# RaphaelHaddad/Real-Time-Brain-Inspired-Video-Memory

Measured on NVIDIA B200. Metric: queries_per_sec_top10_384d, higher is better.
Workload: dtype tf32

## Files before the change

real-time-brain-inspired-video-memory_b200/csrc/common.cuh:

```cuda
#pragma once
#include <cuda_runtime.h>
#include <cuda_bf16.h>
#include <stdint.h>
#include <stdio.h>
#include <math.h>
#include <utility>
#include "../../include/vidmem.h"

namespace vm {

void set_error(const char *fmt, ...);
#define VM_CUDA_CHECK(expr)                                                                      \
    do {                                                                                         \
        cudaError_t _e = (expr);                                                                 \
        if (_e != cudaSuccess) {                                                                 \
            vm::set_error("%s failed: %s (%s:%d)", #expr, cudaGetErrorString(_e), __FILE__, __LINE__); \
            return VM_ERR_CUDA;                                                                  \
        }                                                                                        \
    } while (0)
#define VM_REQUIRE(cond, code, ...)          \
    do {                                     \
        if (!(cond)) {                       \
            vm::set_error(__VA_ARGS__);      \
            return (code);                   \
        }                                    \
    } while (0)

__device__ __forceinline__ void pdl_wait() { asm volatile("griddepcontrol.wait;" ::: "memory"); }
__device__ __forceinline__ void pdl_launch_dependents() { asm volatile("griddepcontrol.launch_dependents;" ::: "memory"); }

template <typename... KArgs, typename... Args>
static inline cudaError_t launch_pdl(void (*kernel)(KArgs...), dim3 grid, dim3 block, size_t smem, cudaStream_t st, bool pdl,
                                     Args &&...args)
{
    cudaLaunchConfig_t cfg = {};
    cfg.gridDim = grid; cfg.blockDim = block; cfg.dynamicSmemBytes = smem; cfg.stream = st;
    cudaLaunchAttribute at[1];
    at[0].id = cudaLaunchAttributeProgrammaticStreamSerialization;
    at[0].val.programmaticStreamSerializationAllowed = 1;
    cfg.attrs = at;
    cfg.numAttrs = pdl ? 1 : 0;
    return cudaLaunchKernelEx(&cfg, kernel, std::forward<Args>(args)...);
}

template <auto Kernel>
static inline cudaError_t max_smem_once(int bytes)
{
    static bool set[64] = {};
    int dev = 0;
    cudaError_t e = cudaGetDevice(&dev);
    if (e != cudaSuccess || set[dev & 63]) return e;
    e = cudaFuncSetAttribute(Kernel, cudaFuncAttributeMaxDynamicSharedMemorySize, bytes);
    if (e == cudaSuccess) set[dev & 63] = true;
    return e;
}

__host__ __device__ __forceinline__ uint32_t f32_ordered(float f)
{
#ifdef __CUDA_ARCH__
    uint32_t b = __float_as_uint(f);
#else
    uint32_t b;
    memcpy(&b, &f, 4);
#endif
    return (b & 0x80000000u) ? ~b : (b | 0x80000000u);
}
__host__ __device__ __forceinline__ float f32_from_ordered(uint32_t o)
{
    uint32_t b = (o & 0x80000000u) ? (o & 0x7FFFFFFFu) : ~o;
#ifdef __CUDA_ARCH__
    return __uint_as_float(b);
#else
    float f;
    memcpy(&f, &b, 4);
    return f;
#endif
}
__host__ __device__ __forceinline__ uint64_t make_key(float score, uint32_t row)
{
    return ((uint64_t)f32_ordered(score) << 32) | (uint64_t)(0xFFFFFFFFu - row);
}
__host__ __device__ __forceinline__ uint32_t key_row(uint64_t k) { return 0xFFFFFFFFu - (uint32_t)(k & 0xFFFFFFFFu); }
__host__ __device__ __forceinline__ float key_score(uint64_t k) { return f32_from_ordered((uint32_t)(k >> 32)); }

static constexpr int SEED_TAB_WORDS = 256 * 64;
#ifdef __CUDACC__
__device__ __forceinline__ float seed_select(const uint32_t *seed_tab, int G, int nq_pad, int q, int k, int lane)
{
    uint32_t vals[8];
#pragma unroll
    for (int t = 0; t < 8; ++t) {
        const int i = lane + 32 * t;
        vals[t] = i < G ? __ldcg(seed_tab + (size_t)i * nq_pad + q) : 0u;
    }
    uint32_t prefix = 0;
    int need = k;
    for (int bit = 31; bit >= 16; --bit) {
        const uint32_t hi = bit == 31 ? 0u : (0xFFFFFFFFu << (bit + 1));
        int cnt = 0;
#pragma unroll
        for (int t = 0; t < 8; ++t) cnt += ((vals[t] & hi) == prefix && ((vals[t] >> bit) & 1u)) ? 1 : 0;
        const int tot = __reduce_add_sync(0xffffffffu, cnt);
        if (tot >= need) prefix |= 1u << bit;
        else need -= tot;
    }
    float sd = f32_from_ordered(prefix);
    if (!(sd > -INFINITY) || G < k) sd = -INFINITY;
    return sd;
}

__device__ __forceinline__ float band_floor(float L, float band)
{
    if (!(L > -INFINITY)) return -INFINITY;
    const float t = __fsub_rd(L, band);
    return nextafterf(t, -INFINITY);
}

#endif

struct RefSum {
    double s, c;
    __device__ __forceinline__ void init() { s = 0.0; c = 0.0; }
    template <bool NEUMAIER>
    __device__ __forceinline__ void add(double x)
    {
        double t = __dadd_rn(s, x);
        if (NEUMAIER) {
            const bool big = fabs(s) >= fabs(x);
            const double hi = big ? s : x, lo = big ? x : s;
            c = __dadd_rn(c, __dadd_rn(__dadd_rn(hi, -t), lo));
        }
        s = t;
    }
    template <bool NEUMAIER>
    __device__ __forceinline__ void add_block(const double (&x)[8])
    {
        double t[8];
        t[0] = __dadd_rn(s, x[0]);
#pragma unroll
        for (int u = 1; u < 8; ++u) t[u] = __dadd_rn(t[u - 1], x[u]);
        if (NEUMAIER) {
#pragma unroll
            for (int u = 0; u < 8; ++u) {
                const double prev = u ? t[u - 1] : s;
                const bool big = fabs(prev) >= fabs(x[u]);
                const double hi = big ? prev : x[u], lo = big ? x[u] : prev;
                c = __dadd_rn(c, __dadd_rn(__dadd_rn(hi, -t[u]), lo));
            }
        }
        s = t[7];
    }
    template <bool NEUMAIER>
    __device__ __forceinline__ double result() const
    {
        double r = s;
        if (NEUMAIER && c != 0.0 && isfinite(c)) r = __dadd_rn(r, c);
        return r;
    }
};

template <bool NEUMAIER, typename F>
__device__ __forceinline__ void ref_sum_range(RefSum &acc, int lo, int hi, F prod)
{
    int i = lo;
    for (; i + 8 <= hi; i += 8) {
        double x[8];
#pragma unroll
        for (int u = 0; u < 8; ++u) x[u] = prod(i + u);
        acc.add_block<NEUMAIER>(x);
    }
    for (; i < hi; ++i) acc.add<NEUMAIER>(prod(i));
}

__device__ __forceinline__ float load_as_float(const float *p, int64_t i) { return p[i]; }
__device__ __forceinline__ float load_as_float(const __nv_bfloat16 *p, int64_t i) { return __bfloat162float(p[i]); }
__device__ __forceinline__ double load_elem(const float *p, int64_t i) { return (double)p[i]; }
__device__ __forceinline__ double load_elem(const __nv_bfloat16 *p, int64_t i) { return (double)__bfloat162float(p[i]); }
__device__ __forceinline__ double load_elem(const double *p, int64_t i) { return p[i]; }
__device__ __forceinline__ double load_as_double(const void *p, int dtype, int64_t i)
{
    if (dtype == VM_F32) return (double)((const float *)p)[i];
    if (dtype == VM_BF16) return (double)__bfloat162float(((const __nv_bfloat16 *)p)[i]);
    return ((const double *)p)[i];
}

static inline int64_t imin64(int64_t a, int64_t b) { return a < b ? a : b; }
static inline int ld_for_dim(int dim) { return (dim + 7) & ~7; }
static inline size_t dtype_size(int dt) { return dt == VM_F32 ? 4 : dt == VM_BF16 ? 2 : 8; }

struct ScanArgs {
    const void *rows;
    const float *inv_norms;
    int dtype;
    int64_t n;
    int dim, ld;
    const float *queries;
    int nq;
    int kp;
    uint64_t *cand;
    int ctas;
    cudaStream_t stream;
    int dump = 0;
    uint64_t *slab = nullptr;
    int *scnt = nullptr;
    uint64_t *ubuf = nullptr;
    int *ucnt = nullptr;
    int ucap = 0;
    float band = 0.0f;
    int ksel = 0;
    int split = 0;
    bool pdl = false;
};
static constexpr int SCAN_UNION_CAP = 16384;
static constexpr int SCAN_SLAB = 128;
static constexpr int SELECT_KEY_CAP = 4096;
static constexpr int SCAN_DUMP_TILE = 128;
static constexpr int SCAN_DUMP_MAX_KEYS = 9472;
int launch_scan_simt(const ScanArgs &a);
int scan_simt_max_queries();
struct ScanCollect {
    const float *thr;
    uint64_t *buf;
    int *cnt;
    int cap;
    const int *pending;
};
struct ScanInfo { int stages = 0, variant = 0; };
int launch_scan_tc(const ScanArgs &a, const void *queries_store_dtype, uint32_t *seed_tab, int *seed_ctr,
                   const ScanCollect *sc = nullptr, ScanInfo *info = nullptr);
bool scan_tc_supported(int dtype, int dim, int nq, int kp, int split = 0);


struct FinalizeArgs {
    int k;
    double min_score;
    int score_mode;
    int64_t row_offset;
    int64_t *out_idx;
    double *out_score;
    int32_t *out_count;
};
struct RescoreArgs {
    const uint64_t *merged;
    int kp;
    const void *rows;
    const float *inv_norms;
    int dtype, ld, dim;
    int64_t n_rows;
    const void *queries;
    int q_dtype, nq;
    double eps;
    int sum_mode;
    FinalizeArgs fin;
    int32_t *flags, *uncertified_count;
    const int *extreme;
    float *collect_thr;
    unsigned long long *cum = nullptr;
};
struct SelectArgs {
    const uint64_t *cand = nullptr;
    int lists = 0, list_len = 0;
    int complete = 0;
    const uint64_t *slab = nullptr;
    const int *scnt = nullptr;
    int ctas = 0;
    const uint64_t *ubuf = nullptr;
    const int *ucnt = nullptr;
    int ucap = 0;
    const uint32_t *seed_tab = nullptr;
    int nq_pad = 0, ksel = 0;
    float band = 0.0f;
};
struct ExactArgs {
    const void *rows;
    const float *inv_norms;
    int dtype, ld, dim;
    int64_t n;
    const void *queries;
    int q_dtype, nq, k, sum_mode;
    int32_t *flags;
    double *xlist_score;
    uint32_t *xlist_row;
    int32_t *xlist_cnt;
    uint8_t *taken;
    int ctas;
    FinalizeArgs fin;
    unsigned long long *cum = nullptr;
    int *done_ctr = nullptr;
};

}
```

real-time-brain-inspired-video-memory_b200/csrc/select.cu:

```cuda
#include "common.cuh"

#include <type_traits>

namespace vm {

static constexpr int MERGE_THREADS = 512;
static constexpr int MERGE_SURV = 1024;

__device__ uint64_t radix_select_kth(const uint64_t *skeys, int total, int kp, int *hist, int *s_bin, int *s_need)
{
    const int tid = threadIdx.x, lane = tid & 31;
    uint64_t prefix = 0;
    int need = kp;
    for (int pass = 0; pass < 8; ++pass) {
        const int shift = 56 - 8 * pass;
        const uint64_t hmask = pass == 0 ? 0ull : (~0ull << (shift + 8));
        if (tid < 256) hist[tid] = 0;
        __syncthreads();
        for (int e = tid; e < total; e += MERGE_THREADS) {
            const uint64_t k = skeys[e];
            const bool act = k != 0 && (k & hmask) == prefix;
            const int bin = act ? (int)((k >> shift) & 0xFF) : -1;
            const unsigned peers = __match_any_sync(__activemask(), bin);
            if (act && (__ffs(peers) - 1) == lane) atomicAdd(&hist[bin], __popc(peers));
// ... 111 lines not shown
            if (nonzero >= kp && k == T) merged[(int64_t)q * kp + kp - 1] = k;
            else merged[(int64_t)q * kp + atomicAdd(&s_m, 1)] = k;
        }
    }
    __syncthreads();
    const int filled = s_m;
    const int last = nonzero >= kp ? kp - 1 : kp;
    for (int e = filled + tid; e < last; e += MERGE_THREADS) merged[(int64_t)q * kp + e] = 0;
}


__device__ __forceinline__ double convert_score(double c, int score_mode)
{
    return score_mode == VM_SCORE_NEO4J ? __ddiv_rn(__dadd_rn(1.0, c), 2.0) : c;
}

template <bool NEUMAIER, typename T>
__device__ double exact_cosine(const void *q, int q_dtype, int64_t qoff, const T *row, int dim)
{
    RefSum dot, qq, rr;
    dot.init(); qq.init(); rr.init();
    for (int i = 0; i < dim; ++i) {
        double x = load_as_double(q, q_dtype, qoff + i);
        double y = load_elem(row, i);
        dot.add<NEUMAIER>(__dmul_rn(x, y));
        qq.add<NEUMAIER>(__dmul_rn(x, x));
        rr.add<NEUMAIER>(__dmul_rn(y, y));
    }
    double n1 = __dsqrt_rn(qq.result<NEUMAIER>());
    double n2 = __dsqrt_rn(rr.result<NEUMAIER>());
    if (n1 == 0.0 || n2 == 0.0) return 0.0;
    return __ddiv_rn(dot.result<NEUMAIER>(), __dmul_rn(n1, n2));
}

template <bool NEUMAIER, typename T>
__device__ double exact_cosine_sq(const double *sq, double n1, const T *row, int dim)
{
    RefSum dot, rr;
    dot.init(); rr.init();
    ref_sum_range<NEUMAIER>(dot, 0, dim, [&](int i) { return __dmul_rn(sq[i], load_elem(row, i)); });
    ref_sum_range<NEUMAIER>(rr, 0, dim, [&](int i) { const double y = load_elem(row, i); return __dmul_rn(y, y); });
    double n2 = __dsqrt_rn(rr.result<NEUMAIER>());
    if (n1 == 0.0 || n2 == 0.0) return 0.0;
    return __ddiv_rn(dot.result<NEUMAIER>(), __dmul_rn(n1, n2));
}

__device__ __forceinline__ bool better(double sa, uint32_t ra, double sb, uint32_t rb)
{
    return sa > sb || (sa == sb && ra < rb);
}

static constexpr int RS_THREADS = 256;
static constexpr int RS_SMEM_ROW_BYTES = 96 * 1024;

__device__ __forceinline__ void load_vec16(const float *p, float *o)
{
    const float4 t = *reinterpret_cast<const float4 *>(p);
    o[0] = t.x; o[1] = t.y; o[2] = t.z; o[3] = t.w;
}
__device__ __forceinline__ void load_vec16(const __nv_bfloat16 *p, float *o)
{
    const uint4 u = *reinterpret_cast<const uint4 *>(p);
    o[0] = __uint_as_float(u.x << 16); o[1] = __uint_as_float(u.x & 0xffff0000u);
    o[2] = __uint_as_float(u.y << 16); o[3] = __uint_as_float(u.y & 0xffff0000u);
    o[4] = __uint_as_float(u.z << 16); o[5] = __uint_as_float(u.z & 0xffff0000u);
    o[6] = __uint_as_float(u.w << 16); o[7] = __uint_as_float(u.w & 0xffff0000u);
}

__device__ __forceinline__ void load_vec16(const double *p, double *o)
{
    const double2 t = *reinterpret_cast<const double2 *>(p);
    o[0] = t.x; o[1] = t.y;
}
template <typename T> struct StageOf { using type = float; };
template <> struct StageOf<double> { using type = double; };

template <bool NEUMAIER, typename T>
__global__ void __launch_bounds__(RS_THREADS, 1) rescore_kernel(const uint64_t *__restrict__ merged, int kp, const T *__restrict__ rows,
                                                            const float *__restrict__ inv_norms, int ld, int dim, int64_t n_rows,
                                                            const void *__restrict__ queries, int q_dtype, double eps,
                                                            FinalizeArgs f, int32_t *__restrict__ flags,
                                                            int32_t *__restrict__ uncertified_count, int chunk,
                                                            const int *__restrict__ extreme, float *__restrict__ collect_thr,
                                                            unsigned long long *__restrict__ cum, const int *__restrict__ incomplete)
{
    constexpr int VEC = 16 / (int)sizeof(T);
    extern __shared__ double rs_smem[];
    double *sq = rs_smem;
    using S = typename StageOf<T>::type;
    S *srow = reinterpret_cast<S *>(rs_smem + chunk);
    const int pitch = chunk + 1;
    __shared__ double s_dot[64], s_rr[64], s_qq;
    __shared__ double s_score[64];
    __shared__ uint32_t s_row[64];
    __shared__ int s_valid[64];
    __shared__ int s_cnt;
    const int q = blockIdx.x, j = threadIdx.x;
    if (j == 0) s_cnt = 0;
    if (j < 64) {
        uint64_t key = j < kp ? merged[(int64_t)q * kp + j] : 0;
        s_valid[j] = key != 0;
        s_row[j] = key != 0 ? key_row(key) : 0;
    }
    __syncthreads();
    const int kind = j < kp ? 0 : (j < 2 * kp ? 1 : (j == 2 * kp ? 2 : 3));
    const int cand = kind == 0 ? j : (kind == 1 ? j - kp : 0);
    const bool active = kind == 2 || (kind < 2 && s_valid[cand]);
    RefSum acc;
    acc.init();
    for (int c0 = 0; c0 < dim; c0 += chunk) {
        const int len = min(chunk, dim - c0);
        const int vlen = (min(chunk, ld - c0) + VEC - 1) / VEC;
        for (int i = j; i < len; i += RS_THREADS) sq[i] = load_as_double(queries, q_dtype, (int64_t)q * dim + c0 + i);
        const int groups = kp * vlen;
        for (int g0 = j; g0 < groups; g0 += 4 * RS_THREADS) {
            S buf[4][VEC];
            int rr_[4], cc_[4];
#pragma unroll
            for (int u = 0; u < 4; ++u) {
                const int g = g0 + u * RS_THREADS;
                rr_[u] = g < groups ? g / vlen : -1;
                cc_[u] = g < groups ? (g - rr_[u] * vlen) * VEC : 0;
                if (rr_[u] >= 0 && s_valid[rr_[u]]) load_vec16(rows + (int64_t)s_row[rr_[u]] * ld + c0 + cc_[u], buf[u]);
                else
#pragma unroll
                    for (int x = 0; x < VEC; ++x) buf[u][x] = (S)0;
            }
#pragma unroll
            for (int u = 0; u < 4; ++u)
                if (rr_[u] >= 0)
#pragma unroll
                    for (int x = 0; x < VEC; ++x)
                        if (cc_[u] + x < chunk) srow[rr_[u] * pitch + cc_[u] + x] = buf[u][x];
        }
        __syncthreads();
        if (active) {
            const S *mine = srow + cand * pitch;
            if (kind == 0)
                ref_sum_range<NEUMAIER>(acc, 0, len, [&](int i) { return __dmul_rn(sq[i], (double)mine[i]); });
            else if (kind == 1)
                ref_sum_range<NEUMAIER>(acc, 0, len, [&](int i) { const double y = (double)mine[i]; return __dmul_rn(y, y); });
            else
                ref_sum_range<NEUMAIER>(acc, 0, len, [&](int i) { const double x = sq[i]; return __dmul_rn(x, x); });
        }
        __syncthreads();
    }
    if (active) {
        const double r = acc.result<NEUMAIER>();
        if (kind == 0) s_dot[cand] = r;
        else if (kind == 1) s_rr[cand] = r;
        else s_qq = r;
    }
    __syncthreads();
    const bool valid = j < 64 && s_valid[j];
    double sc = 0.0;
    const uint32_t row = j < 64 ? s_row[j] : 0;
    if (valid) {
        const double n1 = __dsqrt_rn(s_qq);
        const double n2 = __dsqrt_rn(s_rr[j]);
        sc = (n1 == 0.0 || n2 == 0.0) ? 0.0 : __ddiv_rn(s_dot[j], __dmul_rn(n1, n2));
    }
    if (j < 64) s_score[j] = sc;
    __syncthreads();
    int ncand = 0;
    for (int i = 0; i < 64; ++i) ncand += s_valid[i];
    int rank = 0;
    if (valid)
        for (int i = 0; i < 64; ++i)
            if (s_valid[i] && i != j && better(s_score[i], s_row[i], sc, row)) ++rank;
    double outv = convert_score(sc, f.score_mode);
    bool emit = valid && rank < f.k && outv > f.min_score;
    if (emit) {
        f.out_idx[(int64_t)q * f.k + rank] = (int64_t)row + f.row_offset;
        f.out_score[(int64_t)q * f.k + rank] = outv;
        atomicAdd(&s_cnt, 1);
    }
    __syncthreads();
    if (valid && rank == min(f.k, ncand) - 1) {
        bool cert = true;
        if (ncand >= kp && (int64_t)ncand < n_rows) {
            float worst = key_score(merged[(int64_t)q * kp + kp - 1]);
            cert = ((double)worst + eps) < sc;
        }
        if (incomplete && incomplete[q]) cert = false;
        const bool bound_ok = !(extreme && *extreme != 0);
        if (!bound_ok && (int64_t)ncand < n_rows) cert = false;
        flags[q] = cert ? 0 : (bound_ok ? 1 : 2);
        if (collect_thr) {
            float t = (float)(sc - 2.0 * eps);
            t = nextafterf(nextafterf(t, -INFINITY), -INFINITY);
            collect_thr[q] = (!cert && bound_ok) ? t : INFINITY;
        }
        if (!cert) { atomicAdd(uncertified_count, 1); if (cum) atomicAdd(cum, 1ull); }
    }
    if (ncand == 0 && j == 0) { flags[q] = 0; if (collect_thr) collect_thr[q] = INFINITY; }
    if (j == 0) f.out_count[q] = s_cnt;
    int cnt = s_cnt;
    for (int t = cnt + j; t < f.k; t += RS_THREADS) {
        f.out_idx[(int64_t)q * f.k + t] = -1;
        f.out_score[(int64_t)q * f.k + t] = 0.0;
    }
}

__device__ __forceinline__ void cp_async16(void *smem_dst, const void *gsrc)
{
    asm volatile("cp.async.cg.shared.global [%0], [%1], 16;" ::"r"((uint32_t)__cvta_generic_to_shared(smem_dst)), "l"(gsrc) : "memory");
}
__device__ __forceinline__ void cp_async_commit() { asm volatile("cp.async.commit_group;" ::: "memory"); }
template <int N> __device__ __forceinline__ void cp_async_wait() { asm volatile("cp.async.wait_group %0;" ::"n"(N) : "memory"); }

static constexpr int SR_THREADS = 512;
static constexpr int BAND_CAP_MIN = 1024, BAND_CAP_MAX = 2048;

template <bool NEUMAIER, typename T, int THREADS>
__device__ void band_score_global(const T *__restrict__ rows, int ld, int dim, const double *sq, double n1, int m, double *s_sc, double *s_rr,
                                  const uint32_t *s_row)
{
    const int tid = threadIdx.x;
    const int lines = (ld * (int)sizeof(T) + 127) / 128;
    for (int e = tid; e < m * lines; e += THREADS) {
        const int r = e / lines, l = e - r * lines;
        asm volatile("prefetch.global.L2 [%0];" ::"l"(reinterpret_cast<const char *>(rows + (int64_t)s_row[r] * ld) + (size_t)l * 128));
    }
    for (int t = tid; t < 2 * m; t += THREADS) {
        const int e = t >> 1;
        const T *row = rows + (int64_t)s_row[e] * ld;
        RefSum acc;
        acc.init();
        if (t & 1) {
            ref_sum_range<NEUMAIER>(acc, 0, dim, [&](int i) { const double y = load_elem(row, i); return __dmul_rn(y, y); });
            s_rr[e] = acc.result<NEUMAIER>();
        } else {
            ref_sum_range<NEUMAIER>(acc, 0, dim, [&](int i) { return __dmul_rn(sq[i], load_elem(row, i)); });
            s_sc[e] = acc.result<NEUMAIER>();
        }
    }
    __syncthreads();
    for (int e = tid; e < m; e += THREADS) {
        const double n2 = __dsqrt_rn(s_rr[e]);
        s_sc[e] = (n1 == 0.0 || n2 == 0.0) ? 0.0 : __ddiv_rn(s_sc[e], __dmul_rn(n1, n2));
    }
    __syncthreads();
}

template <int THREADS>
__device__ int band_emit(int m, const double *s_sc, const uint32_t *s_row, int *s_out, const FinalizeArgs &f, int q)
{
    const int tid = threadIdx.x;
    if (tid == 0) *s_out = 0;
    __syncthreads();
    for (int e = tid; e < m; e += THREADS) {
        const double sc = s_sc[e];
        const uint32_t row = s_row[e];
        int rank = 0;
        for (int i = 0; i < m && rank < f.k; ++i) rank += better(s_sc[i], s_row[i], sc, row) ? 1 : 0;
        if (rank < f.k) {
            const double outv = convert_score(sc, f.score_mode);
            if (outv > f.min_score) {
                f.out_idx[(int64_t)q * f.k + rank] = (int64_t)row + f.row_offset;
                f.out_score[(int64_t)q * f.k + rank] = outv;
                atomicMax(s_out, rank + 1);
            }
        }
    }
    __syncthreads();
    const int cntv = *s_out;
    if (tid == 0) f.out_count[q] = cntv;
    for (int t = cntv + tid; t < f.k; t += THREADS) {
        f.out_idx[(int64_t)q * f.k + t] = -1;
        f.out_score[(int64_t)q * f.k + t] = 0.0;
    }
    return cntv;
}

static constexpr uint32_t NO_ROW = 0xFFFFFFFFu;

template <bool NEUMAIER, typename T, int THREADS>
__device__ __forceinline__ void stage_and_chain(const T *__restrict__ rows, int ld, int dim, int kp, const uint32_t *s_rid,
                                                unsigned char *srow, int pitch, const double *sq, double *s_dot, double *s_rr, double *s_qq)
{
    const int tid = threadIdx.x, j = tid;
    const int gpr = ld * (int)sizeof(T) / 16;
    const int c1 = gpr / 3, c2 = 2 * gpr / 3;
#pragma unroll
    for (int c = 0; c < 3; ++c) {
        const int g_lo = c == 0 ? 0 : (c == 1 ? c1 : c2), g_hi = c == 0 ? c1 : (c == 1 ? c2 : gpr);
        const int w = g_hi - g_lo;
        for (int e = tid; e < kp * w; e += THREADS) {
            const int r = e / w, g = g_lo + (e - r * w);
            const uint32_t rid = s_rid[r];
            if (rid != NO_ROW)
                cp_async16(srow + (size_t)r * pitch + (size_t)g * 16,
                           reinterpret_cast<const unsigned char *>(rows + (int64_t)rid * ld) + (size_t)g * 16);
        }
        cp_async_commit();
    }
    const int kind = j < kp ? 0 : (j < 2 * kp ? 1 : ((j == 2 * kp && s_qq != nullptr) ? 2 : 3));
    const int cidx = kind == 0 ? j : (kind == 1 ? j - kp : 0);
    const bool active = kind == 2 || (kind < 2 && s_rid[cidx] != NO_ROW);
    const T *mine = reinterpret_cast<const T *>(srow + (size_t)cidx * pitch);
    constexpr int EPG = 16 / (int)sizeof(T);
    RefSum acc;
    acc.init();
#pragma unroll
    for (int c = 0; c < 3; ++c) {
        if (c == 0) cp_async_wait<2>();
        else if (c == 1) cp_async_wait<1>();
        else cp_async_wait<0>();
        __syncthreads();
        const int g_lo = c == 0 ? 0 : (c == 1 ? c1 : c2), g_hi = c == 0 ? c1 : (c == 1 ? c2 : gpr);
        const int i_lo = g_lo * EPG, i_hi = min(g_hi * EPG, dim);
        if (active) {
            if (kind == 0)
                ref_sum_range<NEUMAIER>(acc, i_lo, i_hi, [&](int i) { return __dmul_rn(sq[i], load_elem(mine, i)); });
            else if (kind == 1)
                ref_sum_range<NEUMAIER>(acc, i_lo, i_hi, [&](int i) { const double y = load_elem(mine, i); return __dmul_rn(y, y); });
            else
                ref_sum_range<NEUMAIER>(acc, i_lo, i_hi, [&](int i) { const double x = sq[i]; return __dmul_rn(x, x); });
        }
    }
    if (active) {
        const double r = acc.result<NEUMAIER>();
        if (kind == 0) s_dot[cidx] = r;
        else if (kind == 1) s_rr[cidx] = r;
        else *s_qq = r;
    }
    __syncthreads();
}

struct SelectSrc {
    const uint64_t *cand;
    int lists, list_len;
    int complete;
    const uint64_t *slab;
    const int *scnt;
    int ctas;
    const uint64_t *ubuf;
    const int *ucnt;
    int ucap;
    const uint32_t *seed_tab;
    int nq_pad, ksel;
    float band;
    int key_cap;
    int band_cap;
};

template <int THREADS>
__device__ int load_slab_keys(const SelectSrc &src, int q, int nq, uint64_t *skeys, int *s_cnts, int *s_total, float *s_bf, bool *incomplete)
{
    const int tid = threadIdx.x, lane = tid & 31, warp = tid >> 5;
    if (warp == 0) {
        float Lb = -INFINITY;
        if (src.seed_tab != nullptr) {
            if (src.ctas >= src.ksel) Lb = seed_select(src.seed_tab, src.ctas, src.nq_pad, q, src.ksel, lane);
            const uint32_t o = __ldcg(src.seed_tab + SEED_TAB_WORDS + q);
            if (o != 0u) Lb = fmaxf(Lb, f32_from_ordered(o));
        }
        if (lane == 0) { *s_bf = band_floor(Lb, src.band); *s_total = 0; }
    }
    for (int c = tid; c < src.ctas; c += THREADS) s_cnts[c] = min(src.scnt[(size_t)c * nq + q], SCAN_SLAB);
    __syncthreads();
    const float bf = *s_bf;
    constexpr int WARPS = THREADS / 32, PER = SCAN_SLAB / 32, BATCH = 4;
    for (int c0 = warp; c0 < src.ctas; c0 += WARPS * BATCH) {
        uint64_t kk[BATCH][PER];
#pragma unroll
        for (int b = 0; b < BATCH; ++b) {
            const int c = c0 + b * WARPS;
            const int cnt = c < src.ctas ? s_cnts[c] : 0;
#pragma unroll
            for (int t = 0; t < PER; ++t)
                kk[b][t] = (lane + 32 * t < cnt) ? __ldcg(src.slab + ((size_t)c * nq + q) * SCAN_SLAB + lane + 32 * t) : 0ull;
        }
#pragma unroll
        for (int b = 0; b < BATCH; ++b)
#pragma unroll
            for (int t = 0; t < PER; ++t) {
                const uint64_t k = kk[b][t];
                if (k != 0 && key_score(k) >= bf) {
                    const int p = atomicAdd(s_total, 1);
                    if (p < src.key_cap) skeys[p] = k;
                }
            }
    }
    const int spilled = src.ucnt[q];
    const int ns = min(spilled, src.ucap);
    for (int e = tid; e < ns; e += THREADS) {
        const uint64_t k = __ldcg(src.ubuf + (size_t)q * src.ucap + e);
        if (k != 0 && key_score(k) >= bf) {
            const int p = atomicAdd(s_total, 1);
            if (p < src.key_cap) skeys[p] = k;
        }
    }
    __syncthreads();
    const int got = *s_total;
    *incomplete = spilled > src.ucap || got > src.key_cap;
    return min(got, src.key_cap);
}

__global__ void __launch_bounds__(SR_THREADS) slab_top_kernel(SelectSrc src, int nq, int kp, uint64_t *__restrict__ merged,
                                                             int *__restrict__ incomplete)
{
    extern __shared__ __align__(16) unsigned char st_smem[];
    uint64_t *skeys = reinterpret_cast<uint64_t *>(st_smem);
    __shared__ int s_cnts[256];
    __shared__ int s_total, s_bin, s_need, s_m;
    __shared__ int hist[256];
    __shared__ float s_bf;
    const int q = blockIdx.x, tid = threadIdx.x;
    bool inc = false;
    const int total = load_slab_keys<SR_THREADS>(src, q, nq, skeys, s_cnts, &s_total, &s_bf, &inc);
    for (int e = tid; e < kp; e += SR_THREADS) merged[(int64_t)q * kp + e] = 0;
    if (tid == 0) { incomplete[q] = inc ? 1 : 0; s_m = 0; }
    __syncthreads();
    if (total <= MERGE_SURV) {
        for (int e = tid; e < total; e += SR_THREADS) {
            const uint64_t k = skeys[e];
            int rank = 0;
            for (int i = 0; i < total; ++i) rank += skeys[i] > k ? 1 : 0;
            if (rank < kp) merged[(int64_t)q * kp + rank] = k;
        }
        return;
    }
    const uint64_t Tk = radix_select_kth(skeys, total, kp, hist, &s_bin, &s_need);
    for (int e = tid; e < total; e += SR_THREADS) {
        const uint64_t k = skeys[e];
        if (k > Tk) merged[(int64_t)q * kp + atomicAdd(&s_m, 1)] = k;
        else if (k == Tk) merged[(int64_t)q * kp + kp - 1] = k;
    }
}

template <bool NEUMAIER, typename T>
__global__ void __launch_bounds__(SR_THREADS, 1) select_rescore_kernel(SelectSrc src, int nq, int kp,
                                                                   const T *__restrict__ rows, int ld, int dim, int64_t n_rows,
                                                                   const void *__restrict__ queries, int q_dtype, double eps,
                                                                   FinalizeArgs f, int32_t *__restrict__ flags,
                                                                   int32_t *__restrict__ uncertified_count,
                                                                   const int *__restrict__ extreme, float *__restrict__ collect_thr,
                                                                   unsigned long long *__restrict__ cum, const float *__restrict__ inv_norms)
{
    extern __shared__ __align__(16) unsigned char sr_smem[];
    uint64_t *skeys = reinterpret_cast<uint64_t *>(sr_smem);
    uint32_t *lmax = reinterpret_cast<uint32_t *>(skeys + src.key_cap);
    double *sq = reinterpret_cast<double *>(lmax + ((src.lists + 3) & ~3));
    const int pitch = ld * (int)sizeof(T) + 16;
    unsigned char *srow = reinterpret_cast<unsigned char *>(sq + ((dim + 1) & ~1));
    double *b_sc = reinterpret_cast<double *>(srow + (((size_t)kp * pitch + 15) & ~(size_t)15));
    uint32_t *b_row = reinterpret_cast<uint32_t *>(b_sc + src.band_cap);
    __shared__ uint64_t s_top[64];
    __shared__ uint32_t s_rid[64];
    __shared__ uint64_t surv[MERGE_SURV];
    __shared__ int hist[256];
    __shared__ int s_bin, s_need, s_m, s_nz, s_cnt, s_band, s_viol, s_out, s_total;
    __shared__ int s_cnts[256];
    __shared__ uint32_t s_L;
    __shared__ float s_thr, s_bf;
    __shared__ double s_dot[64], s_rr[64], s_qq, s_score[64];
    const int q = blockIdx.x, tid = threadIdx.x, lane = tid & 31, warp = tid >> 5;

    pdl_launch_dependents();
    if (tid == 0) { s_m = 0; s_nz = 0; s_cnt = 0; s_band = 0; s_viol = 0; s_thr = -INFINITY; }
    if (tid < 64) s_top[tid] = 0;
    pdl_wait();
    __syncthreads();

    const bool union_mode = src.slab != nullptr;
    int total, lists = src.lists, list_len = src.list_len;
    bool overflow = false;
    int nz = 0;
    if (union_mode) {
        total = load_slab_keys<SR_THREADS>(src, q, nq, skeys, s_cnts, &s_total, &s_bf, &overflow);
        lists = 0;
        if (tid == 0) nz = total;
    } else {
        total = lists * list_len;
#pragma unroll 10
        for (int e = tid; e < total; e += SR_THREADS) {
            const int l = e / list_len, j = e - l * list_len;
            const uint64_t k = src.cand[((int64_t)l * nq + q) * list_len + j];
            skeys[e] = k;
            nz += k != 0;
        }
    }
    for (int i = tid; i < dim; i += SR_THREADS) sq[i] = load_as_double(queries, q_dtype, (int64_t)q * dim + i);
    if (nz) atomicAdd(&s_nz, nz);
    __syncthreads();
    const int nonzero = s_nz;
    bool done = false;
    if (total <= MERGE_SURV) {
        for (int e = tid; e < total; e += SR_THREADS) {
            const uint64_t k = skeys[e];
            if (k == 0) continue;
            int rank = 0;
            for (int i = 0; i < total; ++i) rank += skeys[i] > k ? 1 : 0;
            if (rank < kp) s_top[rank] = k;
        }
        done = true;
    } else if (nonzero >= kp && lists >= kp && lists <= 256) {
        for (int l = warp; l < lists; l += SR_THREADS / 32) {
            uint32_t m = 0;
            for (int j = lane; j < list_len; j += 32) m = max(m, (uint32_t)(skeys[l * list_len + j] >> 32));
            m = __reduce_max_sync(0xffffffffu, m);
            if (lane == 0) lmax[l] = m;
        }
        __syncthreads();
        if (warp == 0) {
            uint32_t vals[8];
#pragma unroll
            for (int t = 0; t < 8; ++t) vals[t] = (lane + 32 * t) < lists ? lmax[lane + 32 * t] : 0u;
            uint32_t prefix = 0;
            int need = kp;
            for (int bit = 31; bit >= 12; --bit) {
                const uint32_t hi = bit == 31 ? 0u : (0xFFFFFFFFu << (bit + 1));
                int cnt = 0;
#pragma unroll
                for (int t = 0; t < 8; ++t) cnt += ((vals[t] & hi) == prefix && ((vals[t] >> bit) & 1u)) ? 1 : 0;
                const int tot = __reduce_add_sync(0xffffffffu, cnt);
                if (tot >= need) prefix |= 1u << bit;
                else need -= tot;
            }
            if (lane == 0) s_L = prefix;
        }
        __syncthreads();
        const uint32_t Lb = s_L;
        if (Lb != 0) {
            for (int e = tid; e < total; e += SR_THREADS) {
                const uint64_t k = skeys[e];
                if ((uint32_t)(k >> 32) >= Lb && k != 0) {
                    const int p = atomicAdd(&s_m, 1);
                    if (p < MERGE_SURV) surv[p] = k;
                }
            }
            __syncthreads();
            const int m = s_m;
            if (m >= kp && m <= MERGE_SURV) {
                for (int e = tid; e < m; e += SR_THREADS) {
                    const uint64_t k = surv[e];
                    int rank = 0;
                    for (int i = 0; i < m; ++i) rank += surv[i] > k ? 1 : 0;
                    if (rank < kp) s_top[rank] = k;
                }
                done = true;
            }
        }
    }
    if (!done) {
        __syncthreads();
        uint64_t Tk = 1;
        if (nonzero >= kp) Tk = radix_select_kth(skeys, total, kp, hist, &s_bin, &s_need);
        if (tid == 0) s_m = 0;
        __syncthreads();
        for (int e = tid; e < total; e += SR_THREADS) {
            const uint64_t k = skeys[e];
            if (k >= Tk && k != 0) {
                if (nonzero >= kp && k == Tk) s_top[kp - 1] = k;
                else s_top[atomicAdd(&s_m, 1)] = k;
            }
        }
    }
    __syncthreads();

    const int j = tid;
    const uint64_t mykey = j < 64 ? s_top[j] : 0;
    const bool cand_valid = j < kp && mykey != 0;
    if (j < 64) s_rid[j] = cand_valid ? key_row(mykey) : NO_ROW;
    __syncthreads();
    stage_and_chain<NEUMAIER, T, SR_THREADS>(rows, ld, dim, kp, s_rid, srow, pitch, sq, s_dot, s_rr, &s_qq);

    double sc = 0.0;
    const uint32_t row = cand_valid ? key_row(mykey) : 0;
    const double n1 = __dsqrt_rn(s_qq);
    if (n1 == 0.0) {
        if (tid == 0) {
            int c = 0;
            const double outv = convert_score(0.0, f.score_mode);
            if (outv > f.min_score)
                for (int64_t r = 0; r < n_rows && c < f.k; ++r)
                    if (__ldg(inv_norms + r) >= 0.0f) {
                        f.out_idx[(int64_t)q * f.k + c] = r + f.row_offset;
                        f.out_score[(int64_t)q * f.k + c] = outv;
                        ++c;
                    }
            for (int t = c; t < f.k; ++t) { f.out_idx[(int64_t)q * f.k + t] = -1; f.out_score[(int64_t)q * f.k + t] = 0.0; }
            f.out_count[q] = c;
            flags[q] = 0;
            if (collect_thr) collect_thr[q] = INFINITY;
        }
        return;
    }
    if (cand_valid) {
        const double n2 = __dsqrt_rn(s_rr[j]);
        sc = (n1 == 0.0 || n2 == 0.0) ? 0.0 : __ddiv_rn(s_dot[j], __dmul_rn(n1, n2));
        if (fabs((double)key_score(mykey) - sc) > eps) atomicAdd(&s_viol, 1);
    }
    if (j < 64) s_score[j] = sc;
    __syncthreads();
    int ncand = 0;
    for (int i = 0; i < kp; ++i) ncand += s_top[i] != 0;
    int rank = 0;
    if (cand_valid)
        for (int i = 0; i < kp; ++i)
            if (s_top[i] != 0 && i != j && better(s_score[i], key_row(s_top[i]), sc, row)) ++rank;
    const double outv = convert_score(sc, f.score_mode);
    const bool emit = cand_valid && rank < f.k && outv > f.min_score;
    if (emit) {
        f.out_idx[(int64_t)q * f.k + rank] = (int64_t)row + f.row_offset;
        f.out_score[(int64_t)q * f.k + rank] = outv;
        atomicAdd(&s_cnt, 1);
    }
    if (cand_valid && ncand >= f.k && rank == f.k - 1) {
        float t = (float)(sc - eps);
        t = nextafterf(nextafterf(t, -INFINITY), -INFINITY);
        s_thr = t;
    }
    __syncthreads();
    const float thr = s_thr;
    {
        int inb = 0;
        for (int e = tid; e < total; e += SR_THREADS) {
            const uint64_t k = skeys[e];
            inb += (k != 0 && key_score(k) >= thr) ? 1 : 0;
        }
        if (inb) atomicAdd(&s_band, inb);
    }
    __syncthreads();
    const int band = s_band;
    const bool bound_ok = !(extreme && *extreme != 0) && s_viol == 0;
    const bool src_complete = union_mode ? !overflow : (src.complete != 0);
    bool cert;
    if (src_complete) cert = band <= ncand;
    else if (union_mode) cert = false;
    else cert = ncand < kp || band < kp;
    if (!bound_ok && (int64_t)ncand < n_rows) cert = false;
    if (ncand == 0) cert = true;
    if (cert) {
        if (tid == 0) {
            flags[q] = 0;
            if (collect_thr) collect_thr[q] = INFINITY;
            f.out_count[q] = s_cnt;
        }
        const int cnt = s_cnt;
        for (int t = cnt + tid; t < f.k; t += SR_THREADS) {
            f.out_idx[(int64_t)q * f.k + t] = -1;
            f.out_score[(int64_t)q * f.k + t] = 0.0;
        }
        return;
    }
    if (tid == 0 && cum) { atomicAdd(cum, 1ull); if (s_viol) atomicAdd(cum + 4, 1ull); }
    if (bound_ok && src_complete && band <= src.band_cap) {
        if (tid == 0) s_m = 0;
        __syncthreads();
        for (int e = tid; e < total; e += SR_THREADS) {
            const uint64_t k = skeys[e];
            if (k != 0 && key_score(k) >= thr) b_row[atomicAdd(&s_m, 1)] = key_row(k);
        }
        __syncthreads();
        for (int b0 = 0; b0 < band; b0 += kp) {
            const int cnt = min(kp, band - b0);
            if (tid < 64) s_rid[tid] = tid < cnt ? b_row[b0 + tid] : NO_ROW;
            __syncthreads();
            stage_and_chain<NEUMAIER, T, SR_THREADS>(rows, ld, dim, kp, s_rid, srow, pitch, sq, s_dot, s_rr, nullptr);
            if (tid < cnt) {
                const double n2 = __dsqrt_rn(s_rr[tid]);
                b_sc[b0 + tid] = (n1 == 0.0 || n2 == 0.0) ? 0.0 : __ddiv_rn(s_dot[tid], __dmul_rn(n1, n2));
            }
            __syncthreads();
        }
        band_emit<SR_THREADS>(band, b_sc, b_row, &s_out, f, q);
        if (tid == 0) {
            flags[q] = 0;
            if (collect_thr) collect_thr[q] = INFINITY;
            if (cum) atomicAdd(cum + 1, 1ull);
        }
        return;
    }
    if (tid == 0) {
        flags[q] = bound_ok ? 1 : 2;
        if (collect_thr) {
            float t = thr > -INFINITY ? (float)((double)thr - eps) : -INFINITY;
            t = nextafterf(t, -INFINITY);
            collect_thr[q] = bound_ok ? t : INFINITY;
        }
        atomicAdd(uncertified_count, 1);
        f.out_count[q] = s_cnt;
    }
    const int cnt = s_cnt;
    for (int t = cnt + tid; t < f.k; t += SR_THREADS) {
        f.out_idx[(int64_t)q * f.k + t] = -1;
        f.out_score[(int64_t)q * f.k + t] = 0.0;
    }
}

static constexpr int CR_THREADS = 512;
template <bool NEUMAIER, typename T>
__global__ void __launch_bounds__(CR_THREADS, 1) collect_rescore_kernel(const uint64_t *__restrict__ buf, const int *__restrict__ cnt, int cap,
                                                                       const T *__restrict__ rows, int ld, int dim,
                                                                       const void *__restrict__ queries, int q_dtype, FinalizeArgs f,
                                                                       int32_t *__restrict__ flags, int32_t *__restrict__ uncertified_count,
                                                                       int nq, unsigned long long *__restrict__ cum, int stage_rows)
{
    extern __shared__ __align__(16) unsigned char cr_smem[];
    double *sq = reinterpret_cast<double *>(cr_smem);
    double *s_sc = sq + ((dim + 1) & ~1);
    double *s_rr = s_sc + cap;
    uint32_t *s_row = reinterpret_cast<uint32_t *>(s_sc + (stage_rows > 0 ? cap : 2 * cap));
    const int pitch = ld * (int)sizeof(T) + 16;
    unsigned char *srow = reinterpret_cast<unsigned char *>(s_row + ((cap + 3) & ~3));
    __shared__ double s_n1;
    __shared__ int s_out;
    __shared__ uint32_t s_rid[64];
    __shared__ double s_dot[64], s_r2[64];
    const int q = blockIdx.x, tid = threadIdx.x;
    if (flags[nq] == 0 || flags[q] != 1) return;
    const int m = cnt[q];
    if (m > cap) {
        if (tid == 0) flags[q] = 2;
        return;
    }
    for (int i = tid; i < dim; i += CR_THREADS) sq[i] = load_as_double(queries, q_dtype, (int64_t)q * dim + i);
    for (int e = tid; e < m; e += CR_THREADS) s_row[e] = key_row(buf[(size_t)q * cap + e]);
    __syncthreads();
    if (tid == 0) {
        RefSum qq; qq.init();
        ref_sum_range<NEUMAIER>(qq, 0, dim, [&](int i) { return __dmul_rn(sq[i], sq[i]); });
        s_n1 = __dsqrt_rn(qq.result<NEUMAIER>());
    }
    __syncthreads();
    if (stage_rows > 0) {
        const double n1 = s_n1;
        for (int b0 = 0; b0 < m; b0 += stage_rows) {
            const int c = min(stage_rows, m - b0);
            if (tid < 64) s_rid[tid] = tid < c ? s_row[b0 + tid] : NO_ROW;
            __syncthreads();
            stage_and_chain<NEUMAIER, T, CR_THREADS>(rows, ld, dim, stage_rows, s_rid, srow, pitch, sq, s_dot, s_r2, nullptr);
            if (tid < c) {
                const double n2 = __dsqrt_rn(s_r2[tid]);
                s_sc[b0 + tid] = (n1 == 0.0 || n2 == 0.0) ? 0.0 : __ddiv_rn(s_dot[tid], __dmul_rn(n1, n2));
            }
            __syncthreads();
        }
    } else {
        band_score_global<NEUMAIER, T, CR_THREADS>(rows, ld, dim, sq, s_n1, m, s_sc, s_rr, s_row);
    }
    band_emit<CR_THREADS>(m, s_sc, s_row, &s_out, f, q);
    if (tid == 0) {
        flags[q] = 0;
        atomicSub(uncertified_count, 1);
        if (cum) atomicAdd(cum + 2, 1ull);
    }
}

#define XK 64

template <int THREADS>
__device__ void exact_merge_query(const double *__restrict__ xlist_score, const uint32_t *__restrict__ xlist_row,
                                  const int32_t *__restrict__ xlist_cnt, int lists, int nq, int k, int q, const FinalizeArgs &f,
                                  uint8_t *__restrict__ taken, double *w_s, uint32_t *w_r, int *w_p, int *s_out)
{
    const int tid = threadIdx.x, lane = tid & 31, warp = tid >> 5;
    const int total = lists * k;
    uint8_t *tk = taken + (int64_t)q * total;
    for (int e = tid; e < total; e += THREADS) tk[e] = 0;
    if (tid == 0) *s_out = 0;
    __syncthreads();
    auto scan_local = [&](double &bs, uint32_t &br, int &bp) {
        bp = -1; bs = 0.0; br = 0;
        for (int e = tid; e < total; e += THREADS) {
            int l = e / k, j = e - l * k;
            if (tk[e] || j >= xlist_cnt[(int64_t)l * nq + q]) continue;
            int64_t g = ((int64_t)l * nq + q) * k + j;
            double s = xlist_score[g];
            uint32_t r = xlist_row[g];
            if (bp < 0 || better(s, r, bs, br)) { bs = s; br = r; bp = e; }
        }
    };
    double bs; uint32_t br; int bp;
    scan_local(bs, br, bp);
    for (int r = 0; r < f.k; ++r) {
        double ms = bs; uint32_t mr = br; int mp = bp;
        for (int o = 16; o > 0; o >>= 1) {
            double ts = __shfl_xor_sync(0xffffffffu, ms, o);
            uint32_t tr = __shfl_xor_sync(0xffffffffu, mr, o);
            int tp = __shfl_xor_sync(0xffffffffu, mp, o);
            if (tp >= 0 && (mp < 0 || better(ts, tr, ms, mr))) { ms = ts; mr = tr; mp = tp; }
        }
        if (lane == 0) { w_s[warp] = ms; w_r[warp] = mr; w_p[warp] = mp; }
        __syncthreads();
// ... 550 lines not shown
```

Measured before the change: 259,700.

## Overlap slab head loads, query staging and L2 prefetch in select kernel

In the slab-union select path, each owner thread now loads the first eight keys of its CTA slab together with the slab count, using vector loads. The block skips the warp-strided slab sweep when no slab is longer than that head. The seed/bound computation moves to the last warp so it overlaps with the slab loads, and the query staging into shared memory is done by otherwise idle threads before the key loading. When few candidates survive, their candidate rows are prefetched into L2 before the exact rescoring, and the rescoring loops are kept rolled to cut code size and register pressure. It adds a requirement that the block has at least 288 threads, plus extra per-thread head registers.

```diff
diff --git a/real-time-brain-inspired-video-memory_b200/csrc/common.cuh b/real-time-brain-inspired-video-memory_b200/csrc/common.cuh
--- a/real-time-brain-inspired-video-memory_b200/csrc/common.cuh
+++ b/real-time-brain-inspired-video-memory_b200/csrc/common.cuh
@@ -159,10 +159,22 @@
     }
 };
 
-template <bool NEUMAIER, typename F>
+template <bool NEUMAIER, bool ROLLED = false, typename F>
 __device__ __forceinline__ void ref_sum_range(RefSum &acc, int lo, int hi, F prod)
 {
     int i = lo;
+    if constexpr (ROLLED) {
+#pragma unroll 1
+        for (; i + 8 <= hi; i += 8) {
+            double x[8];
+#pragma unroll
+            for (int u = 0; u < 8; ++u) x[u] = prod(i + u);
+            acc.add_block<NEUMAIER>(x);
+        }
+#pragma unroll 1
+        for (; i < hi; ++i) acc.add<NEUMAIER>(prod(i));
+        return;
+    }
     for (; i + 8 <= hi; i += 8) {
         double x[8];
 #pragma unroll
diff --git a/real-time-brain-inspired-video-memory_b200/csrc/select.cu b/real-time-brain-inspired-video-memory_b200/csrc/select.cu
--- a/real-time-brain-inspired-video-memory_b200/csrc/select.cu
+++ b/real-time-brain-inspired-video-memory_b200/csrc/select.cu
@@ -437,7 +437,7 @@
     constexpr int EPG = 16 / (int)sizeof(T);
     RefSum acc;
     acc.init();
-#pragma unroll
+#pragma unroll 1
     for (int c = 0; c < 3; ++c) {
         if (c == 0) cp_async_wait<2>();
         else if (c == 1) cp_async_wait<1>();
@@ -447,11 +447,11 @@
         const int i_lo = g_lo * EPG, i_hi = min(g_hi * EPG, dim);
         if (active) {
             if (kind == 0)
-                ref_sum_range<NEUMAIER>(acc, i_lo, i_hi, [&](int i) { return __dmul_rn(sq[i], load_elem(mine, i)); });
+                ref_sum_range<NEUMAIER, true>(acc, i_lo, i_hi, [&](int i) { return __dmul_rn(sq[i], load_elem(mine, i)); });
             else if (kind == 1)
-                ref_sum_range<NEUMAIER>(acc, i_lo, i_hi, [&](int i) { const double y = load_elem(mine, i); return __dmul_rn(y, y); });
+                ref_sum_range<NEUMAIER, true>(acc, i_lo, i_hi, [&](int i) { const double y = load_elem(mine, i); return __dmul_rn(y, y); });
             else
-                ref_sum_range<NEUMAIER>(acc, i_lo, i_hi, [&](int i) { const double x = sq[i]; return __dmul_rn(x, x); });
+                ref_sum_range<NEUMAIER, true>(acc, i_lo, i_hi, [&](int i) { const double x = sq[i]; return __dmul_rn(x, x); });
         }
     }
     if (active) {
@@ -480,11 +480,28 @@
     int band_cap;
 };
 
+static constexpr int SLAB_HEAD = 8;
 template <int THREADS>
 __device__ int load_slab_keys(const SelectSrc &src, int q, int nq, uint64_t *skeys, int *s_cnts, int *s_total, float *s_bf, bool *incomplete)
 {
+    static_assert(THREADS >= 256 + 32, "slab owners and the bound warp must not overlap");
     const int tid = threadIdx.x, lane = tid & 31, warp = tid >> 5;
-    if (warp == 0) {
+    constexpr int WARPS = THREADS / 32;
+    const int spilled = src.ucnt[q];
+    int cnt = 0;
+    uint64_t head[SLAB_HEAD];
+    if (tid < src.ctas) {
+        const ulonglong2 *sl = reinterpret_cast<const ulonglong2 *>(src.slab + ((size_t)tid * nq + q) * SCAN_SLAB);
+        cnt = src.scnt[(size_t)tid * nq + q];
+#pragma unroll
+        for (int h = 0; h < SLAB_HEAD / 2; ++h) {
+            const ulonglong2 v = __ldcg(sl + h);
+            head[2 * h] = v.x; head[2 * h + 1] = v.y;
+        }
+        cnt = min(cnt, SCAN_SLAB);
+        s_cnts[tid] = cnt;
+    }
+    if (warp == WARPS - 1) {
         float Lb = -INFINITY;
         if (src.seed_tab != nullptr) {
             if (src.ctas >= src.ksel) Lb = seed_select(src.seed_tab, src.ctas, src.nq_pad, q, src.ksel, lane);
@@ -493,19 +510,29 @@
         }
         if (lane == 0) { *s_bf = band_floor(Lb, src.band); *s_total = 0; }
     }
-    for (int c = tid; c < src.ctas; c += THREADS) s_cnts[c] = min(src.scnt[(size_t)c * nq + q], SCAN_SLAB);
-    __syncthreads();
+    const bool long_slabs = __syncthreads_or(cnt > SLAB_HEAD);
     const float bf = *s_bf;
-    constexpr int WARPS = THREADS / 32, PER = SCAN_SLAB / 32, BATCH = 4;
-    for (int c0 = warp; c0 < src.ctas; c0 += WARPS * BATCH) {
+    if (tid < src.ctas)
+#pragma unroll
+        for (int h = 0; h < SLAB_HEAD; ++h) {
+            const uint64_t k = head[h];
+            if (h < cnt && k != 0 && key_score(k) >= bf) {
+                const int p = atomicAdd(s_total, 1);
+                if (p < src.key_cap) skeys[p] = k;
+            }
+        }
+    constexpr int PER = (SCAN_SLAB - SLAB_HEAD + 31) / 32, BATCH = 4;
+    for (int c0 = warp; long_slabs && c0 < src.ctas; c0 += WARPS * BATCH) {
         uint64_t kk[BATCH][PER];
 #pragma unroll
         for (int b = 0; b < BATCH; ++b) {
             const int c = c0 + b * WARPS;
-            const int cnt = c < src.ctas ? s_cnts[c] : 0;
+            const int n = c < src.ctas ? s_cnts[c] : 0;
 #pragma unroll
-            for (int t = 0; t < PER; ++t)
-                kk[b][t] = (lane + 32 * t < cnt) ? __ldcg(src.slab + ((size_t)c * nq + q) * SCAN_SLAB + lane + 32 * t) : 0ull;
+            for (int t = 0; t < PER; ++t) {
+                const int e = SLAB_HEAD + lane + 32 * t;
+                kk[b][t] = e < n ? __ldcg(src.slab + ((size_t)c * nq + q) * SCAN_SLAB + e) : 0ull;
+            }
         }
 #pragma unroll
         for (int b = 0; b < BATCH; ++b)
@@ -518,7 +545,6 @@
                 }
             }
     }
-    const int spilled = src.ucnt[q];
     const int ns = min(spilled, src.ucap);
     for (int e = tid; e < ns; e += THREADS) {
         const uint64_t k = __ldcg(src.ubuf + (size_t)q * src.ucap + e);
@@ -603,10 +629,24 @@
     int total, lists = src.lists, list_len = src.list_len;
     bool overflow = false;
     int nz = 0;
+    {
+        const int lo = union_mode ? 256 : 0, hi = union_mode ? SR_THREADS - 32 : SR_THREADS;
+        if (tid >= lo && tid < hi)
+#pragma unroll 4
+            for (int i = tid - lo; i < dim; i += hi - lo) sq[i] = load_as_double(queries, q_dtype, (int64_t)q * dim + i);
+    }
     if (union_mode) {
         total = load_slab_keys<SR_THREADS>(src, q, nq, skeys, s_cnts, &s_total, &s_bf, &overflow);
         lists = 0;
         if (tid == 0) nz = total;
+        if (total <= 4 * kp) {
+            const int lines = (ld * (int)sizeof(T) + 127) / 128;
+            for (int e = tid; e < total * lines; e += SR_THREADS) {
+                const int r = e / lines;
+                asm volatile("prefetch.global.L2 [%0];" ::"l"(reinterpret_cast<const char *>(rows + (int64_t)key_row(skeys[r]) * ld) +
+                                                             (size_t)(e - r * lines) * 128));
+            }
+        }
     } else {
         total = lists * list_len;
 #pragma unroll 10
@@ -617,7 +657,6 @@
             nz += k != 0;
         }
     }
-    for (int i = tid; i < dim; i += SR_THREADS) sq[i] = load_as_double(queries, q_dtype, (int64_t)q * dim + i);
     if (nz) atomicAdd(&s_nz, nz);
     __syncthreads();
     const int nonzero = s_nz;
```

Result: no change. 262,200 (median of 6 runs) (+1.0%).
